# julius-sk/spgemm-prunning

Hardware: AMD Instinct MI355X
Metric: SpGEMM+SSpMM GTEPS (edges/s) & HBM-BW% on Reddit h=256 k=16; vs CPU SpMM (higher is better)
Workload: dtype f32

## Files before the change

spgemm-prunning_amd/csrc/common.h:

```cpp
#pragma once

#include <hip/hip_runtime.h>

#include <atomic>
#include <cstdint>
#include <cstdio>
#include <string>
#include <type_traits>

#include "maxk_hip.h"
#include "token_items.h"

namespace maxk {

constexpr int kWave = 64;
static_assert(kPtrWindow == kWave, "a pointer window holds one entry per lane");
constexpr int kBlock = 256;
constexpr int kWavesPerBlock = kBlock / kWave;
constexpr int kMaxDim = 256;
constexpr int kBucketAccDoubles = 18432;

#ifndef MAXK_FWD_U
#define MAXK_FWD_U 8
#endif
#ifndef MAXK_BWD_U
#define MAXK_BWD_U 8
#endif
#ifndef MAXK_FWD_SHORT
#define MAXK_FWD_SHORT 16
#endif
#ifndef MAXK_FWD_STREAM
#define MAXK_FWD_STREAM 64
#endif
#ifndef MAXK_FWD_RECORDS
#define MAXK_FWD_RECORDS 1
#endif
#ifndef MAXK_FWD_RECORDS_DEEP
#define MAXK_FWD_RECORDS_DEEP 1
#endif
#ifndef MAXK_FWD_WAVES
#define MAXK_FWD_WAVES 1
#endif
#ifndef MAXK_FWD_EMIT_WAVES
#define MAXK_FWD_EMIT_WAVES 1
#endif
#ifndef MAXK_BWD_WAVES
#define MAXK_BWD_WAVES 1
#endif
#ifndef MAXK_XCD_SUM
#define MAXK_XCD_SUM 1
#endif
#ifndef MAXK_XCD_SUM_RUN
#define MAXK_XCD_SUM_RUN 64
#endif
#ifndef MAXK_BWD_X4
#define MAXK_BWD_X4 1
#endif
#ifndef MAXK_X4_U
#define MAXK_X4_U 0
#endif
#ifndef MAXK_PULL_SHIFT_DELTA
#define MAXK_PULL_SHIFT_DELTA 0
#endif
constexpr size_t kPullLdsBytes = 160 * 1024;
__host__ __device__ inline size_t pull_lds_bytes(int ks, int kp, int shift) {
    return ((size_t)ks * 8 + kp) << shift;
}
__host__ __device__ inline bool pull_fits(int ks, int kp, int shift) {
    return pull_lds_bytes(ks, kp, shift) <= kPullLdsBytes;
}
__host__ __device__ inline int pull_ks(int kp, int shift) {
    return pull_fits(kp + 1, kp, shift) ? kp + 1 : kp;
}
#ifndef MAXK_PULL_SHFL
#define MAXK_PULL_SHFL 1
#endif
#ifndef MAXK_PULL_F4_FLUSH
#define MAXK_PULL_F4_FLUSH 1
#endif
#ifndef MAXK_PULL_U
#define MAXK_PULL_U 4
#endif
#ifndef MAXK_PULL_QU
#define MAXK_PULL_QU 2
#endif
#ifndef MAXK_PULL_Q
#define MAXK_PULL_Q 1
#endif
#ifndef MAXK_PULL_H
#define MAXK_PULL_H 16
#endif
#ifndef MAXK_PULL_MIN_KP
#define MAXK_PULL_MIN_KP 8
#endif
#ifndef MAXK_PULL_MIN_KP_WIDE
#define MAXK_PULL_MIN_KP_WIDE 16
#endif
#ifndef MAXK_PULL_TRANSPOSE
#define MAXK_PULL_TRANSPOSE 1
#endif
#ifndef MAXK_PULL_VPL8
#define MAXK_PULL_VPL8 0
#endif
#ifndef MAXK_PACK4
#define MAXK_PACK4 1
#endif
#ifndef MAXK_TOPK_BISECT
#define MAXK_TOPK_BISECT 1
#endif
#ifndef MAXK_TOPK_LB
#define MAXK_TOPK_LB 1
#endif
#ifndef MAXK_PULL_SEL4
#define MAXK_PULL_SEL4 1
#endif
#ifndef MAXK_PULL_XCD
#define MAXK_PULL_XCD 1
#endif
#ifndef MAXK_FWD_XCD
#define MAXK_FWD_XCD 1
#endif
#ifndef MAXK_P1_XCD
#define MAXK_P1_XCD 1
#endif
#ifndef MAXK_CSC_STAGE
#define MAXK_CSC_STAGE 1
#endif
#ifndef MAXK_T_AUX
#define MAXK_T_AUX 2
#endif
#ifndef MAXK_SCATTER_ROWS4
#define MAXK_SCATTER_ROWS4 1
#endif
#ifndef MAXK_TOPK_BLOCKS
#define MAXK_TOPK_BLOCKS 16384
#endif
#ifndef MAXK_P1_ITEMS
#define MAXK_P1_ITEMS 16
#endif
#ifndef MAXK_P2_ITEMS
#define MAXK_P2_ITEMS 16
#endif
#ifndef MAXK_PACK_GRID
#define MAXK_PACK_GRID 4096
#endif
#ifndef MAXK_BUCKET_U
#define MAXK_BUCKET_U 8
#endif
#ifndef MAXK_BUCKET_PARTS
#define MAXK_BUCKET_PARTS 4
#endif
#ifndef MAXK_TOPK_ROWS4
#define MAXK_TOPK_ROWS4 1
#endif
#ifndef MAXK_TOPK_ROWS4_KMAX
#define MAXK_TOPK_ROWS4_KMAX 48
#endif
#ifndef MAXK_TOPK_FENCE_WAIT
#define MAXK_TOPK_FENCE_WAIT 0
#endif
#ifndef MAXK_FWD_OUT_NT
#define MAXK_FWD_OUT_NT 2
#endif
constexpr size_t kInfinityCacheBytes = 256ull << 20;
#ifndef MAXK_BSORT_U
#define MAXK_BSORT_U 2
#endif
#ifndef MAXK_DENSE_ROUTE
#define MAXK_DENSE_ROUTE 1
#endif
#ifndef MAXK_DENSE_DMAX
#define MAXK_DENSE_DMAX 128
#endif
#ifndef MAXK_DENSE_U
#define MAXK_DENSE_U 4
#endif
#ifndef MAXK_DENSE_PICK
#define MAXK_DENSE_PICK 1
#endif
#ifndef MAXK_DENSE_PICK_DMAX
#define MAXK_DENSE_PICK_DMAX 64
#endif
#ifndef MAXK_DENSE_WAVES
#define MAXK_DENSE_WAVES 24
#endif
#ifndef MAXK_CSC_GROUP_DEG
#define MAXK_CSC_GROUP_DEG 16
#endif
#ifndef MAXK_CSC_GROUP_U
#define MAXK_CSC_GROUP_U 4
#endif
#ifndef MAXK_T_LOAD_NT
#define MAXK_T_LOAD_NT 1
#endif
#ifndef MAXK_SUM_U
#define MAXK_SUM_U 0
#endif

void set_error(const char *fmt, ...);
void clear_error();

#define MAXK_REQUIRE(cond, ...)                  \
    do {                                         \
        if (!(cond)) {                           \
            ::maxk::set_error(__VA_ARGS__);      \
            return MAXK_ERR_INVALID;             \
        }                                        \
    } while (0)

#define MAXK_HIP(call)                                                              \
    do {                                                                            \
        hipError_t e_ = (call);                                                     \
        if (e_ != hipSuccess) {                                                     \
            ::maxk::set_error("%s failed: %s", #call, hipGetErrorString(e_));       \
            return MAXK_ERR_HIP;                                                    \
        }                                                                           \
    } while (0)

#define MAXK_LAUNCHED(name)                                                         \
    do {                                                                            \
        hipError_t e_ = hipGetLastError();                                          \
        if (e_ != hipSuccess) {                                                     \
            ::maxk::set_error("%s launch failed: %s", name, hipGetErrorString(e_)); \
            return MAXK_ERR_HIP;                                                    \
        }                                                                           \
    } while (0)

inline hipStream_t as_stream(void *s) { return reinterpret_cast<hipStream_t>(s); }

inline int64_t ceil_div(int64_t a, int64_t b) { return (a + b - 1) / b; }

inline size_t al256(size_t x) { return (x + 255) / 256 * 256; }

template <int V>
using const_t = std::integral_constant<int, V>;
template <int... Vs, class F>
bool with_const(int v, F &&f) {
    return ((v == Vs && (f(const_t<Vs>{}), true)) || ...);
}
template <class F>
bool with_lanes(int v, F &&f) {
    return with_const<1, 2, 4, 8, 16, 32, 64>(v, f);
}
inline int bad_lanes(int lanes) {
    set_error("unsupported lane group %d", lanes);
    return MAXK_ERR_INVALID;
}

inline int64_t device_cus() {
    constexpr int kMaxDevices = 64;
    static std::atomic<int> cache[kMaxDevices] = {};
    int dev = 0;
    if (hipGetDevice(&dev) != hipSuccess || dev < 0 || dev >= kMaxDevices) {
        (void)hipGetLastError();
        return 256;
    }
    int n = cache[dev].load(std::memory_order_relaxed);
    if (n == 0) {
        if (hipDeviceGetAttribute(&n, hipDeviceAttributeMultiprocessorCount, dev) != hipSuccess ||
            n <= 0) {
            (void)hipGetLastError();
            n = 256;
        }
        cache[dev].store(n, std::memory_order_relaxed);
    }
    return n;
}

inline int device_ordinal() {
    int dev = 0;
    if (hipGetDevice(&dev) != hipSuccess || dev < 0) {
        (void)hipGetLastError();
        return 0;
    }
    return dev;
}

inline int lanes_per_edge(int k) {
    int g = 1;
    while (g < k && g < kWave) g <<= 1;
    return g;
}

__device__ __forceinline__ int lane_id() { return __lane_id(); }

__global__ void zero_words_kernel(uint32_t *__restrict__ p, int64_t n);
int zero_words(void *p, int64_t n, hipStream_t s);

bool dense_route(int D, int k);
bool dense_pick(int D, int k);
size_t dense_forward_workspace_size(int64_t num_rows, int64_t num_cols, int64_t num_e, int D,
                                    int chunk);
int dense_forward(const int32_t *row_ptr, const int32_t *col_idx, const float *edge_val,
                  const float *cbsr_val, const uint8_t *cbsr_idx, const float *row_div,
                  float *out, int64_t num_rows, int64_t num_cols, int64_t num_e, int D, int k,
                  int chunk, void *workspace, size_t workspace_bytes, hipStream_t s,
                  int accumulate);

constexpr int kXcds = 8;
inline int64_t xcd_grid(int64_t blocks) { return (blocks + kXcds - 1) / kXcds * kXcds; }
__device__ __forceinline__ int xcd_contiguous_block(int b, int grid) {
    const int per = grid / kXcds;
    return (b % kXcds) * per + b / kXcds;
}
__device__ __forceinline__ int xcd_window_block(int b, int grid, int run) {
    const int w = kXcds * run;
    const int base = b / w * w;
    const int ws = grid - base < w ? grid - base : w;
    return base + xcd_contiguous_block(b - base, ws);
}

__device__ __forceinline__ __amdgpu_buffer_rsrc_t wave_buffer(const void *p, uint32_t bytes) {
    const uint64_t a = reinterpret_cast<uint64_t>(p);
    const uint32_t lo = __builtin_amdgcn_readfirstlane((uint32_t)a);
    const uint32_t hi = __builtin_amdgcn_readfirstlane((uint32_t)(a >> 32));
    return __builtin_amdgcn_make_buffer_rsrc(reinterpret_cast<void *>(((uint64_t)hi << 32) | lo),
                                             0, (int)__builtin_amdgcn_readfirstlane(bytes),
                                             0x00020000);
}

__device__ __forceinline__ void wave_lds_fence() {
    __builtin_amdgcn_fence(__ATOMIC_RELEASE, "wavefront");
    __builtin_amdgcn_wave_barrier();
    __builtin_amdgcn_fence(__ATOMIC_ACQUIRE, "wavefront");
}

namespace {
template <int TAG>
__global__ __launch_bounds__(kBlock) void slab_fixup_kernel(const float *__restrict__ slab,
                                                            const int32_t *__restrict__ slab_row,
                                                            float *__restrict__ out, int width,
                                                            int n_items) {
    const int item = (int)((blockIdx.x * (int64_t)kBlock + threadIdx.x) / 16);
    const int g = threadIdx.x % 16;
    const int grp = (threadIdx.x % kWave) / 16;
    if (item >= n_items) return;
    const int row = slab_row[item];
    if (row < 0 || (item > 0 && slab_row[item - 1] == row)) return;
    int n = 1;
    for (int base = item + 1;; base += 16) {
        const int i = base + g;
        const bool same = i < n_items && slab_row[i] == row;
        const uint32_t mine = (uint32_t)(__ballot(same) >> (16 * grp)) & 0xffffu;
        const int run = __builtin_ctz(~mine | 0x10000u);
        n += run;
        if (run < 16) break;
    }
    float *o = out + (int64_t)row * width;
    const float *sl = slab + (int64_t)item * width;
    if ((width & 3) == 0 && width <= 256) {
        constexpr int SU = 4;
        float4 a[4];
#pragma unroll
        for (int c = 0; c < 4; ++c) {
            const int j = g * 4 + 64 * c;
            a[c] = j < width ? *reinterpret_cast<const float4 *>(o + j) : make_float4(0, 0, 0, 0);
        }
        for (int i0 = 0; i0 < n; i0 += SU) {
            float4 b[SU][4];
#pragma unroll
            for (int u = 0; u < SU; ++u)
#pragma unroll
                for (int c = 0; c < 4; ++c) {
                    const int j = g * 4 + 64 * c;
                    const int i = i0 + u < n ? i0 + u : n - 1;
                    b[u][c] = j < width ? *reinterpret_cast<const float4 *>(sl + (int64_t)i * width + j)
                                        : make_float4(0, 0, 0, 0);
                }
#pragma unroll
            for (int u = 0; u < SU; ++u) {
                if (i0 + u >= n) break;
#pragma unroll
                for (int c = 0; c < 4; ++c) {
                    a[c].x += b[u][c].x;
                    a[c].y += b[u][c].y;
                    a[c].z += b[u][c].z;
                    a[c].w += b[u][c].w;
                }
            }
        }
#pragma unroll
        for (int c = 0; c < 4; ++c) {
            const int j = g * 4 + 64 * c;
            if (j < width) *reinterpret_cast<float4 *>(o + j) = a[c];
        }
    } else {
        for (int j = g; j < width; j += 16) {
            float a = o[j];
            for (int i = 0; i < n; ++i) a += sl[(int64_t)i * width + j];
            o[j] = a;
        }
    }
}
}

template <int TAG>
inline int launch_slab_fixup(const float *slab, const int32_t *slab_row, float *out, int width,
                             int n_items, hipStream_t s) {
    if (n_items <= 0) return MAXK_OK;
    hipLaunchKernelGGL(slab_fixup_kernel<TAG>, dim3((unsigned)ceil_div(n_items, kBlock / 16)),
                       dim3(kBlock), 0, s, slab, slab_row, out, width, n_items);
    MAXK_LAUNCHED("slab_fixup_kernel");
    return MAXK_OK;
}

}
```

spgemm-prunning_amd/csrc/spgemm_fwd.hip:

```cpp
#include "cbsr_pack.h"
#include "common.h"

namespace maxk {
namespace {

inline int fwd_lanes_per_edge(int k, int64_t num_rows, int64_t num_e) {
    const int g = lanes_per_edge(k);
    const int gmin = num_e < kFwdSparseDegree * num_rows ? 16 : 8;
    return g < gmin ? gmin : g;
}

constexpr uint32_t kRecSkip = 0x7fbadbadu;
__global__ __launch_bounds__(kPackBlock) void cbsr_records_kernel(const float *__restrict__ cbsr_val,
                                                                  const uint8_t *__restrict__ cbsr_idx,
                                                                  uint8_t *__restrict__ rec,
                                                                  int num_rows, int k, int D) {
    __shared__ uint32_t s_bits[kPackBlock * 8];
    __shared__ int s_dup[kPackBlock];
    const int tpv = k >> 2;
    const int vpw = kPackBlock / tpv;
    const int t = threadIdx.x;
    const int vl = t / tpv, l0 = (t - vl * tpv) * 4;
    const int RS = 5 * k;
    for (int64_t g0 = (int64_t)blockIdx.x * vpw; g0 < num_rows; g0 += (int64_t)gridDim.x * vpw) {
        const int64_t v = g0 + vl;
        const bool act = vl < vpw && v < num_rows;
        for (int i = t; i < vpw * 8; i += kPackBlock) s_bits[i] = 0u;
        if (t < vpw) s_dup[t] = 0;
        __syncthreads();
        uint32_t w = 0u;
        float o[4] = {0.f, 0.f, 0.f, 0.f};
        if (act) {
            const uint8_t *ci = cbsr_idx + v * k;
            const float *cv = cbsr_val + v * k;
            w = (uint32_t)ci[l0] | ((uint32_t)ci[l0 + 1] << 8) | ((uint32_t)ci[l0 + 2] << 16) |
                ((uint32_t)ci[l0 + 3] << 24);
            uint32_t bad = 0u;
#pragma unroll
            for (int j = 0; j < 4; ++j) {
                o[j] = cv[l0 + j];
                const uint32_t sj = (w >> (8 * j)) & 255u;
                const uint32_t old = atomicOr(&s_bits[vl * 8 + (sj >> 5)], 1u << (sj & 31));
                bad |= ((old >> (sj & 31)) & 1u) | (sj >= (uint32_t)D ? 1u : 0u);
            }
            if (bad) s_dup[vl] = 1;
        }
        __syncthreads();
        if (act) {
            const bool any = s_dup[vl] != 0;
            uint8_t *p = rec + v * RS;
#pragma unroll
            for (int j = 0; j < 4; ++j) {
                const uint32_t sj = (w >> (8 * j)) & 255u;
                float x = o[j];
                bool keep = sj < (uint32_t)D;
                if (any) {
                    const int l = l0 + j;
                    const uint8_t *ci = cbsr_idx + v * k;
                    const float *cv = cbsr_val + v * k;
                    for (int m = 0; m < l; ++m) keep = keep && ci[m] != sj;
                    if (keep)
                        for (int m = l + 1; m < k; ++m)
                            if (ci[m] == sj) x += cv[m];
                }
                const uint32_t xb = __float_as_uint(x);
                const uint32_t ob = !keep ? kRecSkip : (x != x ? 0x7fc00000u : xb);
                reinterpret_cast<uint32_t *>(p)[l0 + j] = ob;
            }
            *reinterpret_cast<uint32_t *>(p + 4 * k + l0) = w;
        }
        __syncthreads();
    }
}

typedef float f32x4 __attribute__((ext_vector_type(4)));

template <int KG, int U, bool WIDE, bool EMIT = false>
struct EdgeWalker {
    static constexpr int G = kWave / KG;

    struct Pending {
        uint32_t b[(U + 3) / 4];
        int pos = -1;
        __device__ __forceinline__ void keep(int u, int sel) {
            const uint32_t x = ((uint32_t)sel & 0xffu) << (8 * (u % 4));
            b[u / 4] = u % 4 == 0 ? x : (b[u / 4] | x);
        }
        __device__ __forceinline__ void flush(__amdgpu_buffer_rsrc_t ers, int ustride, int lane_off,
                                              int lim, int k, int l) const {
#pragma unroll
            for (int u = 0; u < U; ++u) {
                const int e = pos + u * ustride + lane_off;
                const int off = pos >= 0 && e < lim && l < k ? e * k + l : (int)0x80000000;
                __builtin_amdgcn_raw_buffer_store_b8((uint8_t)(b[u / 4] >> (8 * (u % 4))), ers,
                                                     off, 0, MAXK_T_AUX);
            }
        }
    };

    __device__ __forceinline__ static void run_rows(float *acc_g, const int32_t *__restrict__ col_idx,
                                                    const float *__restrict__ edge_val,
                                                    const uint8_t *__restrict__ rec, int RS,
                                                    int e0, int e_end, int sb_g, int len_g,
                                                    int n_it, int k, int trash, int lane,
                                                    uint8_t *__restrict__ esel) {
        const int l0 = lane % KG;
        const int n = e_end - e0;
        const auto crs = wave_buffer(col_idx + e0, (uint32_t)n * 4u);
        const auto vrs = wave_buffer(edge_val + e0, (uint32_t)n * 4u);
        const auto rrs = wave_buffer(rec, 0xffffffffu);
        const int lo = (sb_g - e0) * 4;
        const auto ers = wave_buffer(EMIT ? esel + (size_t)(uint32_t)e0 * k : nullptr,
                                     EMIT ? (uint32_t)n * (uint32_t)k : 0u);
        const int g_off = sb_g - e0;
        for (int it = 0; it < n_it; ++it) {
            int c[U];
            float w[U];
#pragma unroll
            for (int u = 0; u < U; ++u) {
                c[u] = (int)__builtin_amdgcn_raw_buffer_load_b32(crs, lo + (it * U + u) * 4, 0, 0);
                w[u] = __uint_as_float(
                    __builtin_amdgcn_raw_buffer_load_b32(vrs, lo + (it * U + u) * 4, 0, 0));
            }
            for (int lb = 0; lb < k; lb += KG) {
                const int l = lb + l0;
                const bool lok = l < k;
                const uint32_t lc = (uint32_t)(lok ? l : k - 1);
                const uint32_t vo = 4u * lc, so = 4u * (uint32_t)k + 2u * lc;
                float v[U];
                int s[U];
#pragma unroll
                for (int u = 0; u < U; ++u) {
                    const uint32_t ro = __umul24((uint32_t)c[u], (uint32_t)RS);
                    v[u] = __uint_as_float(
                        __builtin_amdgcn_raw_buffer_load_b32(rrs, (int)(ro + vo), 0, 0));
                    s[u] = __builtin_amdgcn_raw_buffer_load_b16(rrs, (int)(ro + so), 0, 0);
                }
#pragma unroll
                for (int u = 0; u < U; ++u) {
                    const bool live = lok && it * U + u < len_g;
                    float *a = &acc_g[live ? min(s[u], trash) : trash];
                    *a = __builtin_fmaf(w[u], v[u], *a);
                    if constexpr (EMIT)
                        __builtin_amdgcn_raw_buffer_store_b8(
                            (uint8_t)s[u], ers, live ? (g_off + it * U + u) * k + l : (int)0x80000000,
                            0, MAXK_T_AUX);
                }
            }
        }
    }

    __device__ __forceinline__ static void run(float *acc_g, const int32_t *__restrict__ col_idx,
                                               const float *__restrict__ edge_val,
                                               const uint8_t *__restrict__ rec, int RS, int sb,
                                               int se, int k, int trash, int lane,
                                               uint8_t *__restrict__ esel) {
        const int grp = lane / KG;
        const int l0 = lane % KG;
        if constexpr (!WIDE) {
            const int n = se - sb;
            const auto crs = wave_buffer(col_idx + sb, (uint32_t)n * 4u);
            const auto vrs = wave_buffer(edge_val + sb, (uint32_t)n * 4u);
            const auto rrs = wave_buffer(rec, 0xffffffffu);
            const auto ers = wave_buffer(EMIT ? esel + (size_t)(uint32_t)sb * k : nullptr,
                                         EMIT ? (uint32_t)n * (uint32_t)k : 0u);
            Pending pend;
            for (int base = 0; base < n; base += G * U) {
                int c[U];
                float w[U];
                const int lo = (base + grp) * 4;
#pragma unroll
                for (int u = 0; u < U; ++u) {
                    c[u] = (int)__builtin_amdgcn_raw_buffer_load_b32(crs, lo + u * G * 4, 0, 0);
                    w[u] = __uint_as_float(
                        __builtin_amdgcn_raw_buffer_load_b32(vrs, lo + u * G * 4, 0, 0));
                }
                if constexpr (EMIT) {
                    pend.flush(ers, G, grp, n, k, l0);
                    __builtin_amdgcn_sched_barrier(0);
                }
                for (int lb = 0; lb < k; lb += KG) {
                    const int l = lb + l0;
                    const bool lok = l < k;
                    const uint32_t lc = (uint32_t)(lok ? l : k - 1);
                    const uint32_t vo = 4u * lc, so = 4u * (uint32_t)k + 2u * lc;
                    float v[U];
                    int s[U];
#pragma unroll
                    for (int u = 0; u < U; ++u) {
                        const uint32_t ro = __umul24((uint32_t)c[u], (uint32_t)RS);
                        v[u] = __uint_as_float(
                            __builtin_amdgcn_raw_buffer_load_b32(rrs, (int)(ro + vo), 0, 0));
                        s[u] = __builtin_amdgcn_raw_buffer_load_b16(rrs, (int)(ro + so), 0, 0);
                    }
#pragma unroll
                    for (int u = 0; u < U; ++u) {
                        const bool live = lok && base + u * G + grp < n;
                        float *a = &acc_g[live ? min(s[u], trash) : trash];
                        *a = __builtin_fmaf(w[u], v[u], *a);
                        if constexpr (EMIT) pend.keep(u, s[u]);
                    }
                    if constexpr (EMIT) pend.pos = base;
                }
            }
            if constexpr (EMIT) pend.flush(ers, G, grp, n, k, l0);
        } else {
            const int last = se - 1;
            for (int base = sb; base < se; base += G * U) {
                int c[U];
                float w[U];
#pragma unroll
                for (int u = 0; u < U; ++u) {
                    const int e = base + u * G + grp;
                    const int ec = e < se ? e : last;
                    c[u] = col_idx[ec];
                    const float wv = edge_val[ec];
                    w[u] = e < se ? wv : 0.f;
                }
                for (int lb = 0; lb < k; lb += KG) {
                    const int l = lb + l0;
                    const bool lok = l < k;
                    const int lc = lok ? l : k - 1;
                    float v[U];
                    int s[U];
#pragma unroll
                    for (int u = 0; u < U; ++u) {
                        const uint8_t *p = rec + (size_t)(uint32_t)c[u] * RS;
                        v[u] = reinterpret_cast<const float *>(p)[lc];
                        s[u] = reinterpret_cast<const uint16_t *>(p + 4 * k)[lc];
                    }
#pragma unroll
                    for (int u = 0; u < U; ++u) {
                        float *a = &acc_g[lok ? min(s[u], trash) : trash];
                        *a = __builtin_fmaf(w[u], v[u], *a);
                    }
                }
            }
        }
    }
};

template <int NC>
__device__ __forceinline__ void flush_row(float *acc, int DS, float *__restrict__ dst, int D,
                                          float div, bool scale, int lane, bool add = false,
                                          bool nt = false) {
    wave_lds_fence();
    if ((D & 3) == 0) {
        for (int j = lane * 4; j < D; j += kWave * 4) {
            float4 a = *reinterpret_cast<float4 *>(&acc[j]);
            *reinterpret_cast<float4 *>(&acc[j]) = make_float4(0.f, 0.f, 0.f, 0.f);
#pragma unroll
            for (int g = 1; g < NC; ++g) {
                float4 *pg = reinterpret_cast<float4 *>(&acc[g * DS + j]);
                const float4 b = *pg;
                a.x += b.x;
                a.y += b.y;
                a.z += b.z;
                a.w += b.w;
                *pg = make_float4(0.f, 0.f, 0.f, 0.f);
            }
            if (scale) {
                a.x = a.x / div;
                a.y = a.y / div;
                a.z = a.z / div;
                a.w = a.w / div;
            }
            if (add) {
                const float4 o = *reinterpret_cast<const float4 *>(&dst[j]);
                a.x += o.x;
                a.y += o.y;
                a.z += o.z;
                a.w += o.w;
            }
            if (nt)
                __builtin_nontemporal_store(
                    __builtin_bit_cast(f32x4, a), reinterpret_cast<f32x4 *>(&dst[j]));
            else
                *reinterpret_cast<float4 *>(&dst[j]) = a;
        }
    } else {
        for (int j = lane; j < D; j += kWave) {
            float a = 0.f;
#pragma unroll
            for (int g = 0; g < NC; ++g) {
                a += acc[g * DS + j];
                acc[g * DS + j] = 0.f;
            }
            dst[j] = (scale ? a / div : a) + (add ? dst[j] : 0.f);
        }
    }
    wave_lds_fence();
}

struct RecordSrc {
    __amdgpu_buffer_rsrc_t rrs;
    uint32_t vo, so, RS;
    __device__ __forceinline__ void load(int c, float &v, int &s) const {
        const uint32_t ro = __umul24((uint32_t)c, RS);
        const uint32_t vb = __builtin_amdgcn_raw_buffer_load_b32(rrs, (int)(ro + vo), 0, 0);
        const int sb = __builtin_amdgcn_raw_buffer_load_b8(rrs, (int)(ro + so), 0, 0);
        v = __uint_as_float(vb);
        s = vb == kRecSkip ? 0x100 : sb;
    }
    __device__ __forceinline__ int col(int s, int D, int trash) const {
        return s < D ? s : trash;
    }
};

template <int KG, int U, class Src>
__device__ __forceinline__ void walk_src(float *acc_g, const int32_t *__restrict__ col_idx,
                                         const float *__restrict__ edge_val, const Src &src,
                                         int sb, int se, int D, int trash, bool lok, int lane) {
    constexpr int G = kWave / KG;
    const int grp = lane / KG;
    const int n = se - sb;
    const auto crs = wave_buffer(col_idx + sb, (uint32_t)n * 4u);
    const auto vrs = wave_buffer(edge_val + sb, (uint32_t)n * 4u);
    for (int base = 0; base < n; base += G * U) {
        int c[U];
        float w[U];
        const int lo = (base + grp) * 4;
#pragma unroll
        for (int u = 0; u < U; ++u) {
            c[u] = (int)__builtin_amdgcn_raw_buffer_load_b32(crs, lo + u * G * 4, 0, 0);
            w[u] = __uint_as_float(__builtin_amdgcn_raw_buffer_load_b32(vrs, lo + u * G * 4, 0, 0));
        }
        float v[U];
        int s[U];
#pragma unroll
        for (int u = 0; u < U; ++u) src.load(c[u], v[u], s[u]);
#pragma unroll
        for (int u = 0; u < U; ++u) {
            const bool live = lok && base + u * G + grp < n;
            float *a = &acc_g[live ? src.col(s[u], D, trash) : trash];
            *a = __builtin_fmaf(w[u], v[u], *a);
        }
    }
}
__device__ __forceinline__ float4 acc_take4(float *a) {
    const float4 x = *reinterpret_cast<float4 *>(a);
    *reinterpret_cast<float4 *>(a) = make_float4(0.f, 0.f, 0.f, 0.f);
    return x;
}
__device__ __forceinline__ void store_out4(float *dst, float4 a, bool scale, float div, bool add,
                                           bool nt) {
    if (scale) {
        a.x = a.x / div;
        a.y = a.y / div;
        a.z = a.z / div;
        a.w = a.w / div;
    }
    if (add) {
        const float4 o = *reinterpret_cast<const float4 *>(dst);
        a.x += o.x;
        a.y += o.y;
        a.z += o.z;
        a.w += o.w;
    }
    if (nt)
        __builtin_nontemporal_store(__builtin_bit_cast(f32x4, a), reinterpret_cast<f32x4 *>(dst));
    else
        *reinterpret_cast<float4 *>(dst) = a;
}

template <int KG, int U, class Src>
__device__ __forceinline__ int stream_rows(float *acc, int DS, int r,
                                           const int32_t *__restrict__ row_ptr, int num_rows,
                                           int64_t d1, const int32_t *__restrict__ col_idx,
                                           const float *__restrict__ edge_val, const Src &src,
                                           const float *__restrict__ row_div,
                                           float *__restrict__ out, int D, int k, int trash,
                                           int lane, int flags, int lmax, int64_t num_e) {
    constexpr int NC = kWave / KG;
    const int g = lane / KG, l0 = lane % KG;
    float *acc_g = acc + g * DS;
    const bool lok = l0 < k;
    const bool add = flags & 1, nt = flags & 2;
    RowHandout<CutHubRows> h(row_ptr, num_rows, r, d1, lmax, lane);
    const int ebase = __builtin_amdgcn_readfirstlane(h.win.v);
    const int64_t span = (num_e - ebase) * 4;
    const auto crs = wave_buffer(col_idx + ebase, (uint32_t)(span < 0xffffffffLL ? span : 0xffffffffLL));
    const auto vrs = wave_buffer(edge_val + ebase, (uint32_t)(span < 0xffffffffLL ? span : 0xffffffffLL));
    int row = -1, e = 0, ee = 0;
    float div = 1.f;
    auto assign = [&]() {
        h.assign<NC>(row < 0, NC, KG, g, lane, [&](int q, int a, int b) {
            row = q;
            e = a;
            ee = b;
            div = row_div ? row_div[q] : 1.f;
        });
    };
    auto load_cw = [&](int (&c)[U], float (&w)[U]) {
#pragma unroll
        for (int u = 0; u < U; ++u) {
            const int off = row >= 0 && e + u < ee ? (e + u - ebase) * 4 : (int)0x80000000;
            c[u] = (int)__builtin_amdgcn_raw_buffer_load_b32(crs, off, 0, 0);
            w[u] = __uint_as_float(__builtin_amdgcn_raw_buffer_load_b32(vrs, off, 0, 0));
        }
    };
    assign();
    int c[U];
    float w[U];
    load_cw(c, w);
    float wn[U];
    while (__ballot(row >= 0)) {
        float v[U];
        int s[U];
#pragma unroll
        for (int u = 0; u < U; ++u) src.load(c[u], v[u], s[u]);
        const int crow = row, ce = e, cee = ee;
        const float cdiv = div;
        const bool fin = crow >= 0 && ce + U >= cee;
        if (fin) row = -1;
        e = ce + U;
        assign();
        load_cw(c, wn);
#pragma unroll
        for (int u = 0; u < U; ++u) {
            const bool live = lok && crow >= 0 && ce + u < cee;
            float *a = &acc_g[live ? src.col(s[u], D, trash) : trash];
            *a = __builtin_fmaf(w[u], v[u], *a);
        }
        if (fin) {
            wave_lds_fence();
            float *dst = out + (int64_t)crow * D;
            for (int j = l0 * 4; j < D; j += KG * 4)
                store_out4(dst + j, acc_take4(acc_g + j), row_div != nullptr, cdiv, add, nt);
            wave_lds_fence();
        }
#pragma unroll
        for (int u = 0; u < U; ++u) w[u] = wn[u];
    }
    return h.next;
}

template <int KG, int U, bool WIDE, bool EMIT, bool STREAM = false>
__global__ __launch_bounds__(kBlock, EMIT ? MAXK_FWD_EMIT_WAVES : MAXK_FWD_WAVES) void spgemm_fwd_kernel(
    const int32_t *__restrict__ row_ptr, const int32_t *__restrict__ col_idx,
    const float *__restrict__ edge_val, const uint8_t *__restrict__ rec, int RS,
    const float *__restrict__ row_div, float *__restrict__ out, float *__restrict__ slab,
    int32_t *__restrict__ slab_row, int num_rows, int64_t num_e, int D, int DS, int k,
    int chunk, int n_items, int accumulate, uint8_t *__restrict__ esel,
    const uint8_t *__restrict__ trec = nullptr) {
    constexpr int NC = kWave / KG;
    extern __shared__ __attribute__((aligned(16))) float lds[];
    const int wid = threadIdx.x / kWave;
    const int lane = lane_id();
    const int blk = MAXK_FWD_XCD ? xcd_contiguous_block(blockIdx.x, gridDim.x) : (int)blockIdx.x;
    const int item = blk * kWavesPerBlock + wid;
    if (item >= n_items) return;
    float *acc = lds + (size_t)wid * NC * DS;
    for (int j = lane * 4; j < NC * DS; j += kWave * 4)
        *reinterpret_cast<float4 *>(&acc[j]) = make_float4(0.f, 0.f, 0.f, 0.f);
    float *acc_g = acc + (lane / KG) * DS;
    const bool lok_s = lane % KG < k;
    auto rec_src = [&]() {
        const uint32_t lc = (uint32_t)(lok_s ? lane % KG : k - 1);
        return RecordSrc{wave_buffer(trec, 0xffffffffu), 4u * lc, 4u * (uint32_t)k + lc,
                         5u * (uint32_t)k};
    };
    const bool tr = (STREAM || MAXK_FWD_RECORDS_DEEP) && !WIDE && !EMIT && trec != nullptr;

    const int64_t total = (int64_t)num_rows + num_e;
    const int64_t d0 = (int64_t)item * chunk;
    const int64_t d1 = d0 + chunk < total ? d0 + chunk : total;
    int r = wave_first_row_token(row_ptr, num_rows, d0);
    const ItemRange it{d0, d1, r, d0 - r};

    int cont = -1;
    if (r > 0) {
        const RowPiece p = cont_piece(CutHubRows{}, it.p_lo, d1, r, row_ptr[r - 1], row_ptr[r], chunk);
        const int64_t sb = p.sb, se = p.se;
        if (sb < se && p.hub) {
            const float div = row_div ? row_div[r - 1] : 1.f;
            wave_lds_fence();
            if (tr)
                walk_src<KG, U>(acc_g, col_idx, edge_val, rec_src(), (int)sb, (int)se, D, DS - 1,
                                lok_s, lane);
            else
                EdgeWalker<KG, U, WIDE, EMIT>::run(acc_g, col_idx, edge_val, rec, RS, (int)sb,
                                                   (int)se, k, DS - 1, lane, esel);
            flush_row<NC>(acc, DS, slab + (int64_t)item * D, D, div, row_div != nullptr, lane);
            cont = r - 1;
        }
    }
    if (lane == 0) slab_row[item] = cont;

    PtrWindow win{row_ptr, num_rows, r, 0};
    constexpr bool BATCH = NC > 1 && !WIDE && !EMIT && !STREAM && MAXK_FWD_SHORT > 0;
    if constexpr (BATCH) win.load(r, lane);
    while (r < num_rows) {
        int64_t rb = row_ptr[r];
        if (!row_owned(d1, r, rb)) break;
        if constexpr (STREAM) {
            if (tr) {
                r = stream_rows<KG, U>(acc, DS, r, row_ptr, num_rows, d1, col_idx, edge_val,
                                       rec_src(), row_div, out, D, k, DS - 1, lane, accumulate,
                                       min(MAXK_FWD_STREAM, chunk), num_e);
            } else {
                const uint32_t lc = (uint32_t)(lok_s ? lane % KG : k - 1);
                const PackedSrc src{wave_buffer(rec, 0xffffffffu), 4u * lc,
                                    4u * (uint32_t)k + 2u * lc, (uint32_t)RS};
                r = stream_rows<KG, U>(acc, DS, r, row_ptr, num_rows, d1, col_idx, edge_val, src,
                                       row_div, out, D, k, DS - 1, lane, accumulate,
                                       min(MAXK_FWD_STREAM, chunk), num_e);
            }
            if (r >= num_rows) break;
            rb = row_ptr[r];
            if (!row_owned(d1, r, rb)) break;
        }
        if (BATCH && !tr) {
            win.slide(r, lane, NC);
            const int rq = r + lane;
            const int rpj = __shfl(win.v, (r - win.wb + lane) & (kWave - 1));
            const int rpn = __shfl_down(rpj, 1);
            const bool okj = lane < NC && rq < num_rows && (int64_t)rq + rpn < d1 &&
                             rpn - rpj <= MAXK_FWD_SHORT;
            const uint64_t bal = __ballot(okj);
            const int m = __builtin_ctzll(~bal);
            if (m >= 2) {
                const int g = lane / KG;
                const int sb_g = __shfl(rpj, g < m ? g : 0);
                const int len_g = g < m ? __shfl(rpn, g) - sb_g : 0;
                const int e0 = __shfl(rpj, 0), e_end = __shfl(rpj, m);
                int maxlen = 0;
                for (int j = 0; j < m; ++j) {
                    const int lj = __shfl(rpn, j) - __shfl(rpj, j);
                    maxlen = lj > maxlen ? lj : maxlen;
                }
                const float divq = row_div && lane < m ? row_div[r + lane] : 1.f;
                wave_lds_fence();
                EdgeWalker<KG, U, WIDE, EMIT>::run_rows(acc_g, col_idx, edge_val, rec, RS, e0,
                                                        e_end, sb_g, len_g, (maxlen + U - 1) / U,
                                                        k, DS - 1, lane, esel);
                for (int j = 0; j < m; ++j) {
                    const float div = __shfl(divq, j);
                    flush_row<1>(acc + j * DS, DS, out + (int64_t)(r + j) * D, D, div,
                                 row_div != nullptr, lane, accumulate & 1, accumulate & 2);
                }
                r += m;
                continue;
            }
        }
        const int64_t se = row_piece(CutHubRows{}, d1, r, rb, row_ptr[r + 1], chunk).se;
        const float div = row_div ? row_div[r] : 1.f;
        wave_lds_fence();
        if (rb < se && tr)
            walk_src<KG, U>(acc_g, col_idx, edge_val, rec_src(), (int)rb, (int)se, D, DS - 1,
                            lok_s, lane);
        else if (rb < se)
            EdgeWalker<KG, U, WIDE, EMIT>::run(acc_g, col_idx, edge_val, rec, RS, (int)rb, (int)se,
                                               k, DS - 1, lane, esel);
        flush_row<NC>(acc, DS, out + (int64_t)r * D, D, div, row_div != nullptr, lane,
                      accumulate & 1, accumulate & 2);
        ++r;
    }
}

int fwd_resident_waves(int kg, int DS, int per_simd) {
    const int by_vgpr = per_simd * 4;
    const size_t per_block = (size_t)kWavesPerBlock * (kWave / kg) * DS * sizeof(float);
    const int by_lds = (int)(kPullLdsBytes / per_block) * kWavesPerBlock;
    return by_lds < by_vgpr ? by_lds : by_vgpr;
}

struct FwdLayout {
    int chunk, n_items, RS, DS, kg;
    bool deep;
    bool stream;
    size_t rec_off, rec_bytes, slab_off, slab_bytes, row_off, total;
};

FwdLayout fwd_layout(int64_t num_rows, int64_t num_cols, int64_t num_e, int D, int k, int chunk,
                     bool emit = false) {
    FwdLayout L{};
    L.RS = record_stride(k, num_cols);
    L.DS = copy_stride(D);
    L.kg = fwd_lanes_per_edge(k, num_rows, num_e);
    const bool narrow = num_cols < (1 << 24) && (uint64_t)num_cols * (uint64_t)L.RS < (1ull << 32);
    L.deep = !emit && num_e >= kFwdSparseDegree * num_rows && narrow;
    L.stream = MAXK_FWD_STREAM > 0 && !emit && narrow && L.kg >= 16 && L.kg <= 32 &&
               D % 4 == 0 && num_e < kFwdSparseDegree * num_rows;
    L.chunk = fwd_chunk(num_rows, num_e, chunk,
                        fwd_resident_waves(L.kg, L.DS, L.deep ? 4 : L.stream ? 5 : 7));
    L.n_items = token_items(num_rows, num_e, L.chunk);
    L.rec_off = 0;
    L.rec_bytes = al256((size_t)num_cols * L.RS);
    L.slab_off = L.rec_off + L.rec_bytes;
    L.slab_bytes = al256((size_t)L.n_items * D * sizeof(float));
    L.row_off = L.slab_off + L.slab_bytes;
    L.total = L.row_off + al256((size_t)L.n_items * sizeof(int32_t));
    return L;
}

template <int KG>
void launch_fwd(const FwdLayout &L, hipStream_t s, const int32_t *row_ptr, const int32_t *col_idx,
                const float *edge_val, const uint8_t *rec, const float *row_div, float *out,
                float *slab, int32_t *slab_row, int num_rows, int64_t num_e, int D, int k,
                int accumulate, uint8_t *esel, const uint8_t *trec = nullptr) {
    constexpr int U = MAXK_FWD_U;
    constexpr int NC = kWave / KG;
    const size_t lds = (size_t)kWavesPerBlock * NC * L.DS * sizeof(float);
    const int64_t blocks = ceil_div(L.n_items, kWavesPerBlock);
    const dim3 grid((unsigned)(MAXK_FWD_XCD ? xcd_grid(blocks) : blocks));
    const int64_t num_cols = (int64_t)(L.rec_bytes / L.RS);
    if (esel)
        hipLaunchKernelGGL((spgemm_fwd_kernel<KG, U, false, true>), grid, dim3(kBlock), lds, s,
                           row_ptr, col_idx, edge_val, rec, L.RS, row_div, out, slab, slab_row,
                           num_rows, num_e, D, L.DS, k, L.chunk, L.n_items, accumulate, esel);
    else if (L.stream) {
        if constexpr (KG >= 16)
            hipLaunchKernelGGL((spgemm_fwd_kernel<KG, U, false, false, true>), grid, dim3(kBlock),
                               lds, s, row_ptr, col_idx, edge_val, rec, L.RS, row_div, out, slab,
                               slab_row, num_rows, num_e, D, L.DS, k, L.chunk, L.n_items,
                               accumulate, nullptr, trec);
    } else if (L.deep)
        hipLaunchKernelGGL((spgemm_fwd_kernel<KG, 2 * U, false, false>), grid, dim3(kBlock), lds,
                           s, row_ptr, col_idx, edge_val, rec, L.RS, row_div, out, slab, slab_row,
                           num_rows, num_e, D, L.DS, k, L.chunk, L.n_items, accumulate, nullptr,
                           trec);
    else if (num_cols < (1 << 24) && L.rec_bytes < (1ull << 32))
        hipLaunchKernelGGL((spgemm_fwd_kernel<KG, U, false, false>), grid, dim3(kBlock), lds, s,
                           row_ptr, col_idx, edge_val, rec, L.RS, row_div, out, slab, slab_row,
                           num_rows, num_e, D, L.DS, k, L.chunk, L.n_items, accumulate, nullptr);
    else
        hipLaunchKernelGGL((spgemm_fwd_kernel<KG, U, true, false>), grid, dim3(kBlock), lds, s,
                           row_ptr, col_idx, edge_val, rec, L.RS, row_div, out, slab, slab_row,
                           num_rows, num_e, D, L.DS, k, L.chunk, L.n_items, accumulate, nullptr);
}

}
}

using namespace maxk;

extern "C" size_t maxk_spgemm_forward_workspace_size(int64_t num_rows, int64_t num_cols,
                                                     int64_t num_e, int32_t dim_origin,
                                                     int32_t dim_k, int32_t chunk_edges) {
    if (num_rows < 0 || num_cols < 0 || num_e < 0 || dim_origin <= 0 || dim_k <= 0) return 0;
    const size_t a = fwd_layout(num_rows, num_cols, num_e, dim_origin, dim_k, chunk_edges).total;
    const size_t b =
        fwd_layout(num_rows, num_cols, num_e, dim_origin, dim_k, chunk_edges, true).total;
    const size_t c = dense_route(dim_origin, dim_k)
                         ? dense_forward_workspace_size(num_rows, num_cols, num_e, dim_origin,
                                                        chunk_edges)
                         : 0;
    return a > b ? (a > c ? a : c) : (b > c ? b : c);
}

namespace {
bool records_ok(const FwdLayout &L, int64_t num_cols, int k) {
    return (L.stream || (MAXK_FWD_RECORDS_DEEP && L.deep)) && k % 4 == 0 && 6 * k > 128 &&
           k <= L.kg && k <= 32 &&
           (uint64_t)num_cols * 5u * (uint64_t)k < (1ull << 32);
}

int forward_impl(const int32_t *row_ptr, const int32_t *col_idx, const float *edge_val,
                 const float *cbsr_val, const uint8_t *cbsr_idx, const float *row_div, float *out,
                 int64_t num_rows, int64_t num_cols, int64_t num_e, int32_t dim_origin,
                 int32_t dim_k, int32_t chunk_edges, void *workspace, size_t workspace_bytes,
                 void *stream, int accumulate, uint8_t *esel = nullptr,
                 const uint8_t *trec = nullptr) {
    MAXK_REQUIRE(num_rows >= 0 && num_rows < (1LL << 31), "num_rows out of range: %lld",
                 (long long)num_rows);
    MAXK_REQUIRE(num_cols >= 0 && num_cols < (1LL << 31), "num_cols out of range");
    MAXK_REQUIRE(num_e >= 0 && num_e < (1LL << 31), "num_e out of range: %lld", (long long)num_e);
    MAXK_REQUIRE(dim_origin >= 1 && dim_origin <= kMaxDim, "dim_origin must be in [1,256], got %d",
                 dim_origin);
    MAXK_REQUIRE(dim_k >= 1 && dim_k <= dim_origin, "dim_k must be in [1,dim_origin], got %d",
                 dim_k);
    MAXK_REQUIRE(chunk_edges >= 0, "chunk_edges must be >= 0");
    MAXK_REQUIRE(num_cols * (int64_t)dim_k < (1LL << 31), "num_cols*k too large");
    if (num_rows == 0) return MAXK_OK;
    MAXK_REQUIRE(row_ptr && out, "row_ptr/out must not be NULL");
    MAXK_REQUIRE(num_e == 0 || (col_idx && edge_val && ((cbsr_val && cbsr_idx) || trec)),
                 "CSR/CBSR pointers must not be NULL");
    MAXK_REQUIRE(num_e == 0 || num_cols > 0, "edges present but num_cols == 0");
    if (!esel && !trec && dense_route(dim_origin, dim_k) && ((uintptr_t)cbsr_val & 15) == 0 &&
        ((uintptr_t)cbsr_idx & 3) == 0 && ((uintptr_t)out & 15) == 0) {
        MAXK_REQUIRE(((uintptr_t)workspace & 255) == 0, "workspace must be 256-B aligned");
        return dense_forward(row_ptr, col_idx, edge_val, cbsr_val, cbsr_idx, row_div, out,
                             num_rows, num_cols, num_e, dim_origin, dim_k, chunk_edges, workspace,
                             workspace_bytes, as_stream(stream), accumulate);
    }
    const FwdLayout L =
        fwd_layout(num_rows, num_cols, num_e, dim_origin, dim_k, chunk_edges, esel != nullptr);
    MAXK_REQUIRE(workspace && workspace_bytes >= L.total,
                 "workspace too small: need %zu bytes, got %zu", L.total, workspace_bytes);
    MAXK_REQUIRE(((uintptr_t)workspace & 255) == 0, "workspace must be 256-B aligned");

    char *ws = reinterpret_cast<char *>(workspace);
    uint8_t *rec = reinterpret_cast<uint8_t *>(ws + L.rec_off);
    float *slab = reinterpret_cast<float *>(ws + L.slab_off);
    int32_t *slab_row = reinterpret_cast<int32_t *>(ws + L.row_off);
    hipStream_t s = as_stream(stream);
    const int D = dim_origin, k = dim_k;
    if (trec) {
        MAXK_REQUIRE(records_ok(L, num_cols, k), "transport records need the streaming forward "
                     "(a sparse graph), k %% 4 == 0 in [24, 32] and num_cols * 5k < 2^32");
    } else if (MAXK_FWD_RECORDS && !esel && num_cols > 0 && records_ok(L, num_cols, k) &&
               ((uintptr_t)cbsr_val & 3) == 0) {
        const int vpw = kPackBlock / (k / 4);
        const int64_t groups = ceil_div(num_cols, (int64_t)vpw);
        hipLaunchKernelGGL(cbsr_records_kernel,
                           dim3((unsigned)(groups < MAXK_PACK_GRID ? groups : MAXK_PACK_GRID)),
                           dim3(kPackBlock), 0, s, cbsr_val, cbsr_idx, rec, (int)num_cols, k, D);
        MAXK_LAUNCHED("cbsr_records_kernel");
        trec = rec;
    } else if (int rc = launch_cbsr_pack(cbsr_val, cbsr_idx, rec, num_cols, k, L.RS, D, L.DS - 1,
                                         s)) {
        return rc;
    }
    const int nr = (int)num_rows;
    const bool big = (double)num_rows * D * 4 > (double)kInfinityCacheBytes;
    const int flags = (accumulate ? 1 : 0) |
                      ((MAXK_FWD_OUT_NT == 1 || (MAXK_FWD_OUT_NT == 2 && big)) ? 2 : 0);
    const bool ok = with_const<8, 16, 32, 64>(L.kg, [&](auto kg_c) {
        launch_fwd<decltype(kg_c)::value>(L, s, row_ptr, col_idx, edge_val, rec, row_div, out,
                                          slab, slab_row, nr, num_e, D, k, flags, esel, trec);
    });
    if (!ok) return bad_lanes(L.kg);
    MAXK_LAUNCHED("spgemm_fwd_kernel");
    return launch_slab_fixup<0>(slab, slab_row, out, D, L.n_items, s);
}
}

extern "C" int maxk_spgemm_forward(const int32_t *row_ptr, const int32_t *col_idx,
                                   const float *edge_val, const float *cbsr_val,
                                   const uint8_t *cbsr_idx, const float *row_div, float *out,
                                   int64_t num_rows, int64_t num_cols, int64_t num_e,
                                   int32_t dim_origin, int32_t dim_k, int32_t chunk_edges,
                                   void *workspace, size_t workspace_bytes, void *stream) {
    clear_error();
    return forward_impl(row_ptr, col_idx, edge_val, cbsr_val, cbsr_idx, row_div, out, num_rows,
                        num_cols, num_e, dim_origin, dim_k, chunk_edges, workspace,
                        workspace_bytes, stream, 0);
}

namespace {
int forward_sel(const int32_t *row_ptr, const int32_t *col_idx, const float *edge_val,
                const float *cbsr_val, const uint8_t *cbsr_idx, const float *row_div, float *out,
                int64_t num_rows, int64_t num_cols, int64_t num_e, int32_t dim_origin,
                int32_t dim_k, int32_t chunk_edges, void *workspace, size_t workspace_bytes,
                void *stream, uint8_t *edge_sel, int accumulate) {
    MAXK_REQUIRE(num_e == 0 || edge_sel, "edge_sel must not be NULL");
    const bool direct = dim_k <= kWave && num_cols < (1 << 24) &&
                        (uint64_t)record_stride(dim_k, num_cols) * (uint64_t)num_cols < (1ull << 32);
    if (int rc = forward_impl(row_ptr, col_idx, edge_val, cbsr_val, cbsr_idx, row_div, out,
                              num_rows, num_cols, num_e, dim_origin, dim_k, chunk_edges, workspace,
                              workspace_bytes, stream, accumulate, direct ? edge_sel : nullptr))
        return rc;
    if (direct || num_e == 0) return MAXK_OK;
    return maxk_edge_selectors(col_idx, cbsr_idx, num_e, dim_k, edge_sel, stream);
}
}

extern "C" int maxk_spgemm_forward_sel(const int32_t *row_ptr, const int32_t *col_idx,
                                       const float *edge_val, const float *cbsr_val,
                                       const uint8_t *cbsr_idx, const float *row_div, float *out,
                                       int64_t num_rows, int64_t num_cols, int64_t num_e,
                                       int32_t dim_origin, int32_t dim_k, int32_t chunk_edges,
                                       void *workspace, size_t workspace_bytes, void *stream,
                                       uint8_t *edge_sel) {
    clear_error();
    return forward_sel(row_ptr, col_idx, edge_val, cbsr_val, cbsr_idx, row_div, out, num_rows,
                       num_cols, num_e, dim_origin, dim_k, chunk_edges, workspace, workspace_bytes,
                       stream, edge_sel, 0);
}

extern "C" int maxk_spgemm_forward_accumulate_sel(
    const int32_t *row_ptr, const int32_t *col_idx, const float *edge_val, const float *cbsr_val,
    const uint8_t *cbsr_idx, const float *row_div, float *out, int64_t num_rows, int64_t num_cols,
    int64_t num_e, int32_t dim_origin, int32_t dim_k, int32_t chunk_edges, void *workspace,
    size_t workspace_bytes, void *stream, uint8_t *edge_sel) {
    clear_error();
    if (num_e == 0) return MAXK_OK;
    return forward_sel(row_ptr, col_idx, edge_val, cbsr_val, cbsr_idx, row_div, out, num_rows,
                       num_cols, num_e, dim_origin, dim_k, chunk_edges, workspace, workspace_bytes,
                       stream, edge_sel, 1);
}

extern "C" int maxk_spgemm_forward_accumulate(const int32_t *row_ptr, const int32_t *col_idx,
                                              const float *edge_val, const float *cbsr_val,
                                              const uint8_t *cbsr_idx, const float *row_div,
                                              float *out, int64_t num_rows, int64_t num_cols,
                                              int64_t num_e, int32_t dim_origin, int32_t dim_k,
                                              int32_t chunk_edges, void *workspace,
                                              size_t workspace_bytes, void *stream) {
    clear_error();
    if (num_e == 0) return MAXK_OK;
    return forward_impl(row_ptr, col_idx, edge_val, cbsr_val, cbsr_idx, row_div, out, num_rows,
                        num_cols, num_e, dim_origin, dim_k, chunk_edges, workspace,
                        workspace_bytes, stream, 1);
}

extern "C" int maxk_records_ok(int64_t num_rows, int64_t num_cols, int64_t num_e,
                               int32_t dim_origin, int32_t dim_k) {
    if (num_rows <= 0 || num_cols <= 0 || num_e <= 0 || dim_origin <= 0 || dim_k <= 0 ||
        dim_k > dim_origin || dim_origin > kMaxDim)
        return 0;
    return records_ok(fwd_layout(num_rows, num_cols, num_e, dim_origin, dim_k, 0), num_cols,
                      dim_k)
               ? 1
               : 0;
}

extern "C" int maxk_cbsr_records(const float *cbsr_val, const uint8_t *cbsr_idx, uint8_t *rec,
                                 int64_t num_rows, int32_t dim_origin, int32_t dim_k,
                                 void *stream) {
    clear_error();
    MAXK_REQUIRE(num_rows >= 0 && num_rows < (1LL << 31), "num_rows out of range");
    MAXK_REQUIRE(dim_origin >= 1 && dim_origin <= kMaxDim, "dim_origin must be in [1,256]");
    MAXK_REQUIRE(dim_k >= 4 && dim_k <= dim_origin && dim_k % 4 == 0 && dim_k <= 128,
                 "transport records need dim_k %% 4 == 0 in [4, min(dim_origin, 128)], got %d",
                 dim_k);
    if (num_rows == 0) return MAXK_OK;
    MAXK_REQUIRE(cbsr_val && cbsr_idx && rec, "pointers must not be NULL");
    MAXK_REQUIRE(((uintptr_t)rec & 3) == 0 && ((uintptr_t)cbsr_val & 3) == 0,
                 "records and values must be 4-B aligned");
    const int vpw = kPackBlock / (dim_k / 4);
    const int64_t groups = ceil_div(num_rows, (int64_t)vpw);
    hipLaunchKernelGGL(cbsr_records_kernel,
                       dim3((unsigned)(groups < MAXK_PACK_GRID ? groups : MAXK_PACK_GRID)),
                       dim3(kPackBlock), 0, as_stream(stream), cbsr_val, cbsr_idx, rec,
                       (int)num_rows, dim_k, dim_origin);
    MAXK_LAUNCHED("cbsr_records_kernel");
    return MAXK_OK;
}

extern "C" int maxk_spgemm_forward_records(const int32_t *row_ptr, const int32_t *col_idx,
                                           const float *edge_val, const uint8_t *rec,
                                           const float *row_div, float *out, int64_t num_rows,
                                           int64_t num_cols, int64_t num_e, int32_t dim_origin,
                                           int32_t dim_k, int32_t chunk_edges, void *workspace,
                                           size_t workspace_bytes, void *stream,
                                           int32_t accumulate) {
    clear_error();
    if (accumulate && num_e == 0) return MAXK_OK;
    MAXK_REQUIRE(num_e == 0 || rec, "rec must not be NULL");
    MAXK_REQUIRE(((uintptr_t)rec & 3) == 0, "records must be 4-B aligned");
    if (num_e == 0) {
        MAXK_REQUIRE(num_rows >= 0 && dim_origin >= 1 && dim_origin <= kMaxDim,
                     "num_rows / dim_origin out of range");
        MAXK_REQUIRE(num_rows == 0 || out, "out must not be NULL");
        return num_rows == 0 ? MAXK_OK
                             : zero_words(out, num_rows * (int64_t)dim_origin, as_stream(stream));
    }
    return forward_impl(row_ptr, col_idx, edge_val, nullptr, nullptr, row_div, out, num_rows,
                        num_cols, num_e, dim_origin, dim_k, chunk_edges, workspace,
                        workspace_bytes, stream, accumulate ? 1 : 0, nullptr, rec);
}
```

Before: 61.48.

## Broadcast edge col/weight batches via DPP row broadcast to cut VGPRs

For lane groups of 16 or more lanes per edge, each lane of a DPP row now loads one (col, weight) pair for a U-step batch, and the values are broadcast with row_bcast DPP instead of every lane holding U copies. The next batch is prefetched one iteration ahead. The change also adds a separate launch-bounds knob for the deep path and raises the assumed per-SIMD waves for KG=64. The aim is to cut per-lane register pressure and redundant loads so more waves stay resident, at the cost of extra DPP instructions and a runtime switch for the broadcast lane.

```diff
diff --git a/spgemm-prunning_amd/csrc/common.h b/spgemm-prunning_amd/csrc/common.h
--- a/spgemm-prunning_amd/csrc/common.h
+++ b/spgemm-prunning_amd/csrc/common.h
@@ -7,6 +7,7 @@
 #include <cstdio>
 #include <string>
 #include <type_traits>
+#include <utility>
 
 #include "maxk_hip.h"
 #include "token_items.h"
@@ -38,8 +39,14 @@
 #ifndef MAXK_FWD_RECORDS_DEEP
 #define MAXK_FWD_RECORDS_DEEP 1
 #endif
+#ifndef MAXK_FWD_DPP
+#define MAXK_FWD_DPP 1
+#endif
 #ifndef MAXK_FWD_WAVES
 #define MAXK_FWD_WAVES 1
+#endif
+#ifndef MAXK_FWD_DEEP_WAVES
+#define MAXK_FWD_DEEP_WAVES 1
 #endif
 #ifndef MAXK_FWD_EMIT_WAVES
 #define MAXK_FWD_EMIT_WAVES 1
@@ -317,6 +324,32 @@
     return __builtin_amdgcn_make_buffer_rsrc(reinterpret_cast<void *>(((uint64_t)hi << 32) | lo),
                                              0, (int)__builtin_amdgcn_readfirstlane(bytes),
                                              0x00020000);
+}
+
+template <int L>
+__device__ __forceinline__ uint32_t row_bcast(uint32_t v) {
+    static_assert(L >= 0 && L < 16, "a DPP row has 16 lanes");
+    return (uint32_t)__builtin_amdgcn_update_dpp(0, (int)v, 0x150 + L, 0xf, 0xf, true);
+}
+__device__ __forceinline__ uint32_t row_bcast(uint32_t v, int l) {
+    switch (l & 15) {
+    case 0: return row_bcast<0>(v);
+    case 1: return row_bcast<1>(v);
+    case 2: return row_bcast<2>(v);
+    case 3: return row_bcast<3>(v);
+    case 4: return row_bcast<4>(v);
+    case 5: return row_bcast<5>(v);
+    case 6: return row_bcast<6>(v);
+    case 7: return row_bcast<7>(v);
+    case 8: return row_bcast<8>(v);
+    case 9: return row_bcast<9>(v);
+    case 10: return row_bcast<10>(v);
+    case 11: return row_bcast<11>(v);
+    case 12: return row_bcast<12>(v);
+    case 13: return row_bcast<13>(v);
+    case 14: return row_bcast<14>(v);
+    default: return row_bcast<15>(v);
+    }
 }
 
 __device__ __forceinline__ void wave_lds_fence() {
diff --git a/spgemm-prunning_amd/csrc/spgemm_fwd.hip b/spgemm-prunning_amd/csrc/spgemm_fwd.hip
--- a/spgemm-prunning_amd/csrc/spgemm_fwd.hip
+++ b/spgemm-prunning_amd/csrc/spgemm_fwd.hip
@@ -75,6 +75,51 @@
 
 typedef float f32x4 __attribute__((ext_vector_type(4)));
 
+template <int KG, int U>
+struct BatchCW {
+    static constexpr int G = kWave / KG;
+    static constexpr bool kDpp = MAXK_FWD_DPP && KG >= 16;
+    static_assert(!kDpp || U <= 16, "a DPP row holds 16 steps");
+    uint32_t c[kDpp ? 1 : U], w[kDpp ? 1 : U];
+    uint32_t r;
+    uint32_t cn, wn, slot;
+    __device__ __forceinline__ void first(__amdgpu_buffer_rsrc_t crs, __amdgpu_buffer_rsrc_t vrs,
+                                          int lane) {
+        if constexpr (kDpp) {
+            const int i = lane % 16;
+            slot = i < U ? (uint32_t)(i * G + lane / KG) * 4u : 0x80000000u;
+            cn = __builtin_amdgcn_raw_buffer_load_b32(crs, (int)slot, 0, 0);
+            wn = __builtin_amdgcn_raw_buffer_load_b32(vrs, (int)slot, 0, 0);
+        }
+    }
+    __device__ __forceinline__ void next(__amdgpu_buffer_rsrc_t crs, __amdgpu_buffer_rsrc_t vrs,
+                                         int base, int lane, uint32_t RS) {
+        if constexpr (kDpp) {
+            c[0] = cn;
+            w[0] = wn;
+            r = __umul24(cn, RS);
+            const uint32_t off = (uint32_t)(base + G * U) * 4u + slot;
+            cn = __builtin_amdgcn_raw_buffer_load_b32(crs, (int)off, 0, 0);
+            wn = __builtin_amdgcn_raw_buffer_load_b32(vrs, (int)off, 0, 0);
+        } else {
+            const int lo = (base + lane / KG) * 4;
+#pragma unroll
+            for (int u = 0; u < U; ++u) {
+                c[u] = __builtin_amdgcn_raw_buffer_load_b32(crs, lo + u * G * 4, 0, 0);
+                w[u] = __builtin_amdgcn_raw_buffer_load_b32(vrs, lo + u * G * 4, 0, 0);
+            }
+        }
+    }
+    __device__ __forceinline__ uint32_t rec(int u, uint32_t RS) const {
+        if constexpr (kDpp) return row_bcast(r, u);
+        else return __umul24(c[u], RS);
+    }
+    __device__ __forceinline__ float weight(int u) const {
+        if constexpr (kDpp) return __uint_as_float(row_bcast(w[0], u));
+        else return __uint_as_float(w[u]);
+    }
+};
+
 template <int KG, int U, bool WIDE, bool EMIT = false>
 struct EdgeWalker {
     static constexpr int G = kWave / KG;
@@ -165,16 +210,10 @@
             const auto ers = wave_buffer(EMIT ? esel + (size_t)(uint32_t)sb * k : nullptr,
                                          EMIT ? (uint32_t)n * (uint32_t)k : 0u);
             Pending pend;
+            BatchCW<KG, U> cw;
+            cw.first(crs, vrs, lane);
             for (int base = 0; base < n; base += G * U) {
-                int c[U];
-                float w[U];
-                const int lo = (base + grp) * 4;
-#pragma unroll
-                for (int u = 0; u < U; ++u) {
-                    c[u] = (int)__builtin_amdgcn_raw_buffer_load_b32(crs, lo + u * G * 4, 0, 0);
-                    w[u] = __uint_as_float(
-                        __builtin_amdgcn_raw_buffer_load_b32(vrs, lo + u * G * 4, 0, 0));
-                }
+                cw.next(crs, vrs, base, lane, (uint32_t)RS);
                 if constexpr (EMIT) {
                     pend.flush(ers, G, grp, n, k, l0);
                     __builtin_amdgcn_sched_barrier(0);
@@ -188,7 +227,7 @@
                     int s[U];
 #pragma unroll
                     for (int u = 0; u < U; ++u) {
-                        const uint32_t ro = __umul24((uint32_t)c[u], (uint32_t)RS);
+                        const uint32_t ro = cw.rec(u, (uint32_t)RS);
                         v[u] = __uint_as_float(
                             __builtin_amdgcn_raw_buffer_load_b32(rrs, (int)(ro + vo), 0, 0));
                         s[u] = __builtin_amdgcn_raw_buffer_load_b16(rrs, (int)(ro + so), 0, 0);
@@ -197,7 +236,7 @@
                     for (int u = 0; u < U; ++u) {
                         const bool live = lok && base + u * G + grp < n;
                         float *a = &acc_g[live ? min(s[u], trash) : trash];
-                        *a = __builtin_fmaf(w[u], v[u], *a);
+                        *a = __builtin_fmaf(cw.weight(u), v[u], *a);
                         if constexpr (EMIT) pend.keep(u, s[u]);
                     }
                     if constexpr (EMIT) pend.pos = base;
@@ -296,7 +335,9 @@
     __amdgpu_buffer_rsrc_t rrs;
     uint32_t vo, so, RS;
     __device__ __forceinline__ void load(int c, float &v, int &s) const {
-        const uint32_t ro = __umul24((uint32_t)c, RS);
+        load_at(__umul24((uint32_t)c, RS), v, s);
+    }
+    __device__ __forceinline__ void load_at(uint32_t ro, float &v, int &s) const {
         const uint32_t vb = __builtin_amdgcn_raw_buffer_load_b32(rrs, (int)(ro + vo), 0, 0);
         const int sb = __builtin_amdgcn_raw_buffer_load_b8(rrs, (int)(ro + so), 0, 0);
         v = __uint_as_float(vb);
@@ -316,24 +357,19 @@
     const int n = se - sb;
     const auto crs = wave_buffer(col_idx + sb, (uint32_t)n * 4u);
     const auto vrs = wave_buffer(edge_val + sb, (uint32_t)n * 4u);
+    BatchCW<KG, U> cw;
+    cw.first(crs, vrs, lane);
     for (int base = 0; base < n; base += G * U) {
-        int c[U];
-        float w[U];
-        const int lo = (base + grp) * 4;
-#pragma unroll
-        for (int u = 0; u < U; ++u) {
-            c[u] = (int)__builtin_amdgcn_raw_buffer_load_b32(crs, lo + u * G * 4, 0, 0);
-            w[u] = __uint_as_float(__builtin_amdgcn_raw_buffer_load_b32(vrs, lo + u * G * 4, 0, 0));
-        }
+        cw.next(crs, vrs, base, lane, src.RS);
         float v[U];
         int s[U];
 #pragma unroll
-        for (int u = 0; u < U; ++u) src.load(c[u], v[u], s[u]);
+        for (int u = 0; u < U; ++u) src.load_at(cw.rec(u, src.RS), v[u], s[u]);
 #pragma unroll
         for (int u = 0; u < U; ++u) {
             const bool live = lok && base + u * G + grp < n;
             float *a = &acc_g[live ? src.col(s[u], D, trash) : trash];
-            *a = __builtin_fmaf(w[u], v[u], *a);
+            *a = __builtin_fmaf(cw.weight(u), v[u], *a);
         }
     }
 }
@@ -435,8 +471,14 @@
     return h.next;
 }
 
+constexpr int fwd_min_waves(int U, bool WIDE, bool EMIT, bool STREAM) {
+    return EMIT                                  ? MAXK_FWD_EMIT_WAVES
+           : !STREAM && !WIDE && U > MAXK_FWD_U ? MAXK_FWD_DEEP_WAVES
+                                                 : MAXK_FWD_WAVES;
+}
+
 template <int KG, int U, bool WIDE, bool EMIT, bool STREAM = false>
-__global__ __launch_bounds__(kBlock, EMIT ? MAXK_FWD_EMIT_WAVES : MAXK_FWD_WAVES) void spgemm_fwd_kernel(
+__global__ __launch_bounds__(kBlock, fwd_min_waves(U, WIDE, EMIT, STREAM)) void spgemm_fwd_kernel(
     const int32_t *__restrict__ row_ptr, const int32_t *__restrict__ col_idx,
     const float *__restrict__ edge_val, const uint8_t *__restrict__ rec, int RS,
     const float *__restrict__ row_div, float *__restrict__ out, float *__restrict__ slab,
@@ -565,6 +607,8 @@
     return by_lds < by_vgpr ? by_lds : by_vgpr;
 }
 
+inline int fwd_deep_per_simd(int kg) { return kg == kWave ? 5 : 4; }
+
 struct FwdLayout {
     int chunk, n_items, RS, DS, kg;
     bool deep;
@@ -583,7 +627,10 @@
     L.stream = MAXK_FWD_STREAM > 0 && !emit && narrow && L.kg >= 16 && L.kg <= 32 &&
                D % 4 == 0 && num_e < kFwdSparseDegree * num_rows;
     L.chunk = fwd_chunk(num_rows, num_e, chunk,
-                        fwd_resident_waves(L.kg, L.DS, L.deep ? 4 : L.stream ? 5 : 7));
+                        fwd_resident_waves(L.kg, L.DS,
+                                           L.deep     ? fwd_deep_per_simd(L.kg)
+                                           : L.stream ? 5
+                                                      : 7));
     L.n_items = token_items(num_rows, num_e, L.chunk);
     L.rec_off = 0;
     L.rec_bytes = al256((size_t)num_cols * L.RS);
```

Result: no change. 61.79 (median of 6 runs) (+0.5%).
